# gersteinlab/REPIC-copy

Hardware: AMD Instinct MI355X
Metric: micrographs/sec (get_cliques, whole node) at 1/2/4/8 MI355X; % HBM roofline (higher is better)
Workload: dtype f64; 1 GPU; C2: {'k': 3, 'n_true': 300, 'box': 180, 'width': 4096, 'height': 4096, 'keep': 0.9, 'jit': 0.08, 'fp': 0.1}; micrographs_per_gpu=10000, scaling=weak, k=3, box_size=180, boxes_per_gpu=9030947, edges_per_gpu=11401310, cliques_per_gpu=5244495, parallelism=dp1 (micrograph shards), io=HBM-resident, steps_in_flight=3, streams=3

## Files before the change

repic-copy_amd/csrc/rgc_abi.cpp:

```cpp
#include <hip/hip_runtime_api.h>

#include <algorithm>
#include <climits>
#include <cstdio>
#include <cstdlib>
#include <cstring>
#include <string>
#include <map>
#include <mutex>
#include <thread>
#include <tuple>
#include <vector>

#include "../../include/repic_gc.h"
#include "pyset.h"
#include "rgc_kernels.h"

using namespace rgc;

static thread_local std::string g_err;

static int fail(const std::string& msg) {
  g_err = msg;
  return -1;
// ... 1 lines not shown
#define HIPCHK(expr)                                                                   \
  do {                                                                                 \
    hipError_t e_ = (expr);                                                            \
    if (e_ != hipSuccess)                                                              \
      return fail(std::string(#expr) + ": " + hipGetErrorString(e_));                   \
  } while (0)
#define TRY(expr)           \
  do {                      \
    int r_ = (expr);        \
    if (r_ != 0) return r_; \
  } while (0)

namespace {

enum DevBufId {
  D_FBOXOFF, D_FIDBASE, D_MGLIST, D_MGOUT, D_CURSOR, D_X, D_Y, D_S,
  D_ROWS, D_W, D_CONF, D_CONS, D_MEMBERS, D_ORDER,
  D_SUBMG, D_SUBX, D_SUBY, D_SUBS, D_ORIG, D_STAMPS,
  D_BOXOFF, D_CELLOFF, D_P0OFF, D_IDBASE, D_GRID, D_CELLSTART, D_SX, D_SY, D_SBOX, D_SPICK, D_SMG, D_BMG,
  D_BPICK, D_FWDCNT, D_FWDOFF, D_TILES, D_TOTAL, D_EDST, D_EJI, D_PARENT, D_HASEDGE, D_CSIZE,
  D_STAT, D_INSKEY, D_COMPMIN, D_CCOUNT, D_COFF, D_INCL, D_VLIST, D_VSORT, D_VROW, D_BOFF, D_RLO, D_ADJG, D_RBOUND, D_RFLAG, D_DFSMG, D_ROOTBOX, D_EXLIST,
  D_LCNT, D_LOFF, D_LROOT0, D_LROOT1, D_LM0, D_LM1, D_LP0, D_LP1, D_PK,
  D_QG, D_QGSLOT,
  D_TIES,
  D_EU, D_EV, D_EJIOUT,
  D_SC_BOX, D_SC_GOFF, D_SC_POFF, D_SC_TP, D_SC_TR, D_SC_TW, D_SC_CNT,
  D_IL_CPTR, D_IL_ROW, D_IL_W, D_IL_REP, D_IL_PAR, D_IL_ROOT, D_IL_CSIZE, D_IL_RCNT, D_IL_RCUR,
  D_IL_RPTR, D_IL_RCOLS, D_IL_CID, D_IL_CN, D_IL_COFF, D_IL_CCUR, D_IL_MEM, D_IL_LOC, D_IL_SCR,
  D_IL_BIG, D_IL_NBIG, D_IL_WSCR, D_IL_X, D_IL_EX, D_IL_RLOC, D_IL_CERT, D_IL_KEY, D_IL_ST,
  D_IL_RMAX, D_IL_OWN, D_IL_LAM, D_IL_GRAD, D_IL_CS, D_IL_CNT, D_IL_GAP, D_IL_STSAVE,
  D_IL_FS, D_IL_FSCNT, D_IL_FSKEEP, D_LBUCKET, D_WIDELIST,
  D_PK_META, D_PK_COLMG, D_PK_SEL, D_PK_SELCNT, D_PK_PRIMAL, D_PK_OFF, D_PK_X, D_PK_PX, D_PK_PY,
  D_PK_PCONF, D_PK_PCOL, D_PK_CONF, D_PK_CX, D_PK_CY,
  D_COUNT
};
enum HostBufId {
  H_FSTAGE, H_STAGE, H_TOTAL, H_MGOUT, H_STAT, H_MGOFF, H_ROWS, H_W, H_CONF, H_CONS, H_MEMBERS,
  H_ORDER, H_EU, H_EV, H_EJIOUT,
  H_PK_META, H_PK_MG, H_PK_PX, H_PK_PY, H_PK_PCONF, H_PK_PCOL, H_COUNT
};

struct Buf {
  void* p = nullptr;
  size_t cap = 0;
};

constexpr int LDS_BLOCK = 1280;
// ... 123 lines not shown
  std::string pend_err;
  int64_t fix_fetch_bytes = 0;
};

static int ensure_dev(rgc_ctx* c, int id, size_t bytes, size_t keep = 0) {
  Buf& b = c->d[id];
  if (bytes == 0) bytes = 16;
  if (b.cap >= bytes) return 0;
  size_t cap = std::max(bytes, b.cap + b.cap / 2);
  cap = (cap + 255) & ~(size_t)255;
  void* p = nullptr;
  HIPCHK(hipMalloc(&p, cap));
  if (b.p && keep) {
    HIPCHK(hipMemcpyAsync(p, b.p, std::min(keep, b.cap), hipMemcpyDeviceToDevice, c->stream));
    HIPCHK(hipStreamSynchronize(c->stream));
  }
  if (b.p) HIPCHK(hipFree(b.p));
  b.p = p;
  b.cap = cap;
  if (id == D_TILES) {
    HIPCHK(hipMemsetAsync(p, 0, cap, c->stream));
    c->tiles_epoch = scan_epoch_count();
  }
  return 0;
}

static int tiles_refresh(rgc_ctx* c) {
  Buf& b = c->d[D_TILES];
  if (!b.p || scan_epoch_count() - c->tiles_epoch < SCAN_EPOCH_REFRESH) return 0;
  HIPCHK(hipMemsetAsync(b.p, 0, b.cap, c->stream));
  c->tiles_epoch = scan_epoch_count();
  return 0;
}

constexpr int QG_BYTES = 1 << 20;
static int ensure_qg(rgc_ctx* c, FusedArgs& A, int k, int nt) {
  A.qg_base = nullptr;
  A.qg_slots = nullptr;
  A.qg_nslots = 0;
  A.qg_bytes = 0;
  if (nt != 1024 || k != 4) return 0;
  if (!c->qg_nslots) {
    int ncu = 0;
    HIPCHK(hipDeviceGetAttribute(&ncu, hipDeviceAttributeMultiprocessorCount, c->device));
    const int ns = (2 * std::max(ncu, 1) + 31) / 32 * 32;
    TRY(ensure_dev(c, D_QG, (size_t)ns * QG_BYTES));
// ... 44 lines not shown
                          bool multi) {
  TRY(ensure_dev(c, D_ROWS, need * k * 4, keep * k * 4));
  TRY(ensure_dev(c, D_W, need * 4, keep * 4));
  TRY(ensure_dev(c, D_CONF, need * 4, keep * 4));
  TRY(ensure_dev(c, D_CONS, need * 4, keep * 4));
  TRY(ensure_dev(c, D_TIES, need * (4 + k) * 4));
  if (members) TRY(ensure_dev(c, D_MEMBERS, need * k * 4, keep * k * 4));
  if (multi) TRY(ensure_dev(c, D_ORDER, need * k, keep * k));
  return 0;
}

static int ensure_edges(rgc_ctx* c, int64_t need, int64_t keep) {
  TRY(ensure_dev(c, D_EU, need * 4, keep * 4));
  TRY(ensure_dev(c, D_EV, need * 4, keep * 4));
  TRY(ensure_dev(c, D_EJIOUT, need * 8, keep * 8));
  return 0;
}

struct FusedIo {
  unsigned long long *cur, *clear;
  const unsigned long long* h_cur;
  int slot;
  MgOut o;
};
static int fused_io(rgc_ctx* c, int n_mg, size_t cur_off, FusedIo* io) {
  TRY(ensure_host(c, H_MGOUT, cur_off + 2 * CUR_BYTES));
  TRY(ensure_dev(c, D_MGOUT, cur_off + 2 * CUR_BYTES));
  char* d = D<char>(c, D_MGOUT);
  if (c->slots_at != d || c->slots_off != cur_off) {
    HIPCHK(hipMemsetAsync(d + cur_off, 0, 2 * CUR_BYTES, c->stream));
    c->slots_at = d;
    c->slots_off = cur_off;
    c->cur_slot = 0;
  }
  const int sl = c->cur_slot;
  io->slot = sl;
  io->cur = reinterpret_cast<unsigned long long*>(d + cur_off + sl * CUR_BYTES);
  io->clear = reinterpret_cast<unsigned long long*>(d + cur_off + (1 - sl) * CUR_BYTES);
  io->h_cur = reinterpret_cast<const unsigned long long*>(H<char>(c, H_MGOUT) + cur_off +
                                                           sl * CUR_BYTES);
  io->o = mgout_bind(d, n_mg);
  return 0;
}

static int run_multi(rgc_ctx* c, int n_mg, int k, double B, double two_b2, int get_cc, int multi,
                     bool want_members, bool want_ji, const int64_t* box_off, const int64_t* id_base, const double* x,
                     const double* y, const double* sc, int64_t out_base,
                     std::vector<MgStat>& st_out, int64_t* C_out, int64_t* E_out) {
  const int64_t N = box_off[(int64_t)n_mg * k];
  const size_t nbo = (size_t)n_mg * k + 1;
  std::vector<int32_t> cell_off(n_mg + 1);
  int64_t cells = 0;
  bool bin_wide = false;
  int max_n = 0;
  for (int m = 0; m < n_mg; ++m) {
    const int64_t nm = box_off[(int64_t)(m + 1) * k] - box_off[(int64_t)m * k];
    bin_wide |= nm > 65535;
    max_n = std::max<int>(max_n, (int)std::min<int64_t>(nm, INT32_MAX));
  }
  for (int m = 0; m < n_mg; ++m) {
    cell_off[m] = (int32_t)cells;
    const int64_t nm = box_off[(int64_t)(m + 1) * k] - box_off[(int64_t)m * k];
    cells += bin_budget(nm, bin_wide) + 2;
  }
// ... 391 lines not shown
      if (want_edges) TRY(ensure_edges(c, c->cap_edges, 0));
      FusedIo io;
      TRY(fused_io(c, n_mg, cur_off, &io));
      if (attempt > 0) HIPCHK(hipMemsetAsync(io.cur, 0, CUR_BYTES, s));
      h_cur = io.h_cur;
      FusedArgs A{};
      A.k = k; A.flags = get_cc | (multi << 1) | (want_members ? 32 : 0);
      A.B = B; A.two_b2 = two_b2;
      A.box_off = d_bo; A.id_base = d_id;
      A.x = x; A.y = y; A.score = sc; A.o = io.o;
      A.cursor = io.cur; A.cap = c->cap_cliques;
      A.cursor_clear = io.clear;
      A.rows = D<int32_t>(c, D_ROWS); A.w = D<float>(c, D_W); A.conf = D<float>(c, D_CONF);
      A.consensus = D<int32_t>(c, D_CONS);
      A.members = want_members ? D<int32_t>(c, D_MEMBERS) : nullptr;
      A.order = multi ? D<uint8_t>(c, D_ORDER) : nullptr;
      A.stamps = nullptr;
      A.eu = want_edges ? D<int32_t>(c, D_EU) : nullptr;
      A.ev = want_edges ? D<int32_t>(c, D_EV) : nullptr;
      A.eji = want_edges ? D<double>(c, D_EJIOUT) : nullptr;
      A.ecap_out = c->cap_edges;
      A.tie_list = D<int32_t>(c, D_TIES);
      A.tie_cap = c->cap_cliques;
      A.esum_n = 0;
      A.wide_list = nullptr;
      A.mg_count = nullptr;
      int64_t ties_done = 0;
#ifdef RGC_STAMPS
      TRY(ensure_dev(c, D_STAMPS, 3 * (size_t)n_mg * rgc::STAMP_SLOTS * 8));
      HIPCHK(hipMemsetAsync(D<void>(c, D_STAMPS), 0, 3 * (size_t)n_mg * rgc::STAMP_SLOTS * 8, s));
#endif
      std::vector<int32_t> todo = todo0, left;
      int ml_off = 0;
      bool overflow = false;
      for (int pass = 0; pass < 3 && (!todo.empty() || (pass == 0 && all0)); ++pass) {
        const bool wide = pass > 0;
        const bool single = pass == 0 && all0;
        std::vector<int> keys;
        std::vector<std::vector<int32_t>> lists;
        left.clear();
        if (single) {
          keys.assign(1, fused_class(nmaxb));
          lists.assign(1, std::vector<int32_t>());
        }
        int last = -1;
        for (int32_t m : todo) {
          const int cl = mg_class(m);
          if (!cl || !plan_of(pass, cl).nmax) { left.push_back(m); continue; }
          if (last < 0 || keys[last] != cl) {
            last = -1;
// ... 17 lines not shown
            HIPCHK(hipMemcpyAsync(D<int32_t>(c, D_MGLIST) + ml_off, f_ml + ml_off, by.size() * 4,
                                  hipMemcpyHostToDevice, s));
        }
        for (size_t q = 0; q < keys.size(); ++q) {
          const FusedPlan& pl = plan_of(pass, keys[q]);
          A.nmax = pl.nmax;
          A.ecap = pl.ecap;
          A.mg_list = single ? nullptr : D<int32_t>(c, D_MGLIST) + ml_off + starts[q];
#ifdef RGC_STAMPS
          A.stamps = D<unsigned long long>(c, D_STAMPS) + (size_t)(ml_off + starts[q]) * rgc::STAMP_SLOTS;
#endif
          TRY(ensure_qg(c, A, k, pl.nt));
          TRY(mark(c, "k_fused"));
          const int le = launch_fused(s, single ? n_mg : (int)lists[q].size(), pl.lds, A, wide,
                                      pl.nt);
          if (le != 0)
            return fail(std::string("fused kernel launch failed (k=") + std::to_string(k) +
                        (wide ? ", f64" : ", f32") + " layout, nmax " + std::to_string(pl.nmax) +
                        ", lds " + std::to_string(pl.lds) + ", " +
                        std::to_string(pl.nt) + " threads): " +
                        (le > 0 ? hipGetErrorString((hipError_t)le) : "unsupported k"));
        }
        TRY(mark(c, "k_fused_ties"));
        if (launch_fused_ties(s, A, ties_done) != 0) return fail("tie kernel launch failed");
        TRY(mark(c, "d2h_stats"));
        HIPCHK(hipMemcpyAsync(H<void>(c, H_MGOUT), D<void>(c, D_MGOUT), cur_off + 2 * CUR_BYTES,
                              hipMemcpyDeviceToHost, s));
        if (c->timing) {
          if (!c->ev_tail) HIPCHK(hipEventCreate(&c->ev_tail));
          HIPCHK(hipEventRecord(c->ev_tail, s));
        }
        HIPCHK(hipGetLastError());
        HIPCHK(hipStreamSynchronize(s));
        const int32_t* fst = ho.status;
        ties_done = std::min<int64_t>((int64_t)h_cur[rgc::CUR_TIES], A.tie_cap);
        ml_off += (int)by.size();
        todo.clear();
        auto check = [&](int32_t m) {
          const int stt = fst[m];
          if (stt == RGC_ST_OVERFLOW) overflow = true;
          else if (stt == RGC_ST_DEFER_WIDE || stt == RGC_ST_DEFER) todo.push_back(m);
        };
        if (single) {
          for (int32_t m = 0; m < n_mg; ++m)
            if (fst[m] >= RGC_ST_DEFER) check(m);
        } else {
          for (const int32_t m : by) check(m);
        }
        for (int32_t m : left) todo.push_back(m);
      }
      fused_total = (int64_t)h_cur[0];
      c->cur_slot = 1 - c->cur_slot;
#ifdef RGC_STAMPS
      const size_t n0w = all0 ? (size_t)n_mg : todo0.size();
      c->stamps.resize(n0w * rgc::STAMP_SLOTS);
      HIPCHK(hipMemcpy(c->stamps.data(), D<void>(c, D_STAMPS), n0w * rgc::STAMP_SLOTS * 8,
                       hipMemcpyDeviceToHost));
#endif
// ... 229 lines not shown
  if (c->cap_cliques < 4096) c->cap_cliques = std::max<int64_t>(4096, N);
  TRY(ensure_outputs(c, c->cap_cliques, 0, k, want_members, multi));
  FusedIo io;
  TRY(fused_io(c, n_mg, cur_off, &io));
  FusedArgs A{};
  A.k = k;
  A.flags = ((flags & RGC_F_GET_CC) ? 1 : 0) | (multi ? 2 : 0) | (want_members ? 32 : 0);
  A.B = (double)in->box_size;
  A.two_b2 = (double)(2 * in->box_size * in->box_size);
  A.box_off = in->dev_box_off; A.id_base = in->dev_id_base;
  A.x = in->x; A.y = in->y; A.score = in->score;
  A.o = io.o;
  A.cursor = io.cur; A.cap = c->cap_cliques;
  A.cursor_clear = io.clear;
  A.rows = D<int32_t>(c, D_ROWS); A.w = D<float>(c, D_W); A.conf = D<float>(c, D_CONF);
  A.consensus = D<int32_t>(c, D_CONS);
  A.members = want_members ? D<int32_t>(c, D_MEMBERS) : nullptr;
  A.order = multi ? D<uint8_t>(c, D_ORDER) : nullptr;
  A.stamps = nullptr;
  A.eu = nullptr; A.ev = nullptr; A.eji = nullptr; A.ecap_out = 0;
  A.mg_list = nullptr;
  A.tie_list = D<int32_t>(c, D_TIES);
  A.tie_cap = c->cap_cliques;
  A.esum_n = n_mg;
  A.mg_count = nullptr;
  const FusedPlan* pw = c->wide_hint ? &cached_plan(k, 1, fused_class(nmaxb)) : nullptr;
  if (pw && !pw->nmax) pw = nullptr;
  A.wide_list = nullptr;
  if (pw) {
    TRY(ensure_dev(c, D_WIDELIST, (size_t)n_mg * 4));
    A.wide_list = D<int32_t>(c, D_WIDELIST);
  }
#ifdef RGC_STAMPS
  return 0;
#endif
  int32_t* d_ml = nullptr;
  if (grp.size() > 1) {
    TRY(ensure_host(c, H_FSTAGE, (size_t)n_mg * 4));
    TRY(ensure_dev(c, D_MGLIST, (size_t)n_mg * 4));
    int32_t* h_ml = H<int32_t>(c, H_FSTAGE);
    size_t o = 0;
    for (const auto& g : grp) {
      std::memcpy(h_ml + o, g.mg.data(), g.mg.size() * 4);
      o += g.mg.size();
    }
    d_ml = D<int32_t>(c, D_MGLIST);
// ... 13 lines not shown
    if (le != 0) return fail("fused kernel launch failed (submit): " +
                             std::string(le > 0 ? hipGetErrorString((hipError_t)le) : "unsupported k"));
  }
  if (pw) {
    FusedArgs Aw = A;
    Aw.mg_list = A.wide_list;
    Aw.mg_count = io.cur + 5;
    Aw.wide_list = nullptr;
    Aw.nmax = pw->nmax;
    Aw.ecap = pw->ecap;
    TRY(ensure_qg(c, Aw, k, pw->nt));
    TRY(mark(c, "k_fused"));
    const int le = launch_fused(s, n_mg, pw->lds, Aw, true, pw->nt);
    if (le != 0) return fail("fused f64 kernel launch failed (submit): " +
                             std::string(le > 0 ? hipGetErrorString((hipError_t)le) : "unsupported k"));
  }
  const bool stats_in_ties = !(flags & RGC_F_LAZY_STATS) && A.tie_list && A.tie_cap > 0;
  if (stats_in_ties) {
    A.stats_dev = D<char>(c, D_MGOUT);
    A.host_stats = H<char>(c, H_MGOUT);
    A.stats_bytes = (int64_t)cur_off;
  }
  TRY(mark(c, "k_fused_ties"));
  if (launch_fused_ties(s, A, 0) != 0) return fail("tie kernel launch failed (submit)");
  c->pend_slot = io.slot;
  c->cur_slot = 1 - c->cur_slot;
  if (c->timing) {
    if (!c->ev_tail) HIPCHK(hipEventCreate(&c->ev_tail));
    HIPCHK(hipEventRecord(c->ev_tail, s));
  }
  if (!c->ev_sub) HIPCHK(hipEventCreateWithFlags(&c->ev_sub, hipEventDisableTiming));
  if (stats_in_ties || (flags & RGC_F_LAZY_STATS)) {
    const size_t so = cur_off + (size_t)io.slot * CUR_BYTES;
    HIPCHK(hipMemcpyAsync(H<char>(c, H_MGOUT) + so, D<char>(c, D_MGOUT) + so, CUR_BYTES,
                          hipMemcpyDeviceToHost, s));
    HIPCHK(hipEventRecord(c->ev_sub, s));
  } else {
    if (!c->copy_set) {
      TRY(shared_copy_stream(c->device, &c->copy_stream));
      c->copy_set = true;
    }
    if (!c->ev_k) HIPCHK(hipEventCreateWithFlags(&c->ev_k, hipEventDisableTiming));
    HIPCHK(hipEventRecord(c->ev_k, s));
    HIPCHK(hipStreamWaitEvent(c->copy_stream, c->ev_k, 0));
    HIPCHK(hipMemcpyAsync(H<void>(c, H_MGOUT), D<void>(c, D_MGOUT), cur_off + 2 * CUR_BYTES,
                          hipMemcpyDeviceToHost, c->copy_stream));
    HIPCHK(hipEventRecord(c->ev_sub, c->copy_stream));
// ... 973 lines not shown
```

repic-copy_amd/csrc/rgc_fused.hip:

```cpp
#pragma clang fp contract(off)

#include <type_traits>

#ifdef RGC_STAMPS
#include <hip/hip_runtime.h>
namespace rgc {
__shared__ unsigned long long g_bwait[16];
__device__ __forceinline__ void raw_barrier() {
  __builtin_amdgcn_fence(__ATOMIC_RELEASE, "workgroup");
  __builtin_amdgcn_s_barrier();
  __builtin_amdgcn_fence(__ATOMIC_ACQUIRE, "workgroup");
}
__device__ __forceinline__ void timed_barrier() {
  const unsigned long long t0 = __builtin_amdgcn_s_memtime();
  raw_barrier();
  if ((threadIdx.x & 63) == 0) g_bwait[threadIdx.x >> 6] += __builtin_amdgcn_s_memtime() - t0;
}
}
#define __syncthreads() ::rgc::timed_barrier()
#endif

#include "rgc_device.h"
#include "rgc_kernels.h"

// ... 1 lines not shown

constexpr int MAXW = 16;
constexpr int fused_rb(int nt) { return nt <= 256 ? 4 : nt >= 1024 ? 5 : 2; }
constexpr int fused_rq(int nt) { return nt >= 1024 ? 0 : fused_rb(nt); }
constexpr int fused_rv(int nt) { return nt >= 1024 ? 0 : fused_rb(nt); }

struct FusedHdr {
  union {
    struct {
      double redd[MAXW];
      int64_t red64[MAXW];
      uint64_t redu[MAXW];
      int redi[MAXW];
    };
    double red4[4][MAXW];
  };
  double minx, miny, cell, inv_cell, inv_celly;
  double xbs;
  float inv_gy;
  int gx, gy, ncell, nkey;
  int E, nodes, cc_cnt, cc_max, target, V, status;
  uint32_t ccur;
  int tief[2];
  int qslot;
  int64_t C, base;
};

__host__ __device__ inline int fused_cells(int nmax) { return nmax <= 2048 ? 4 * nmax : 2 * nmax; }

__host__ __device__ inline int fwd_blocks(int nmax) { return (nmax + 63) / 64; }

__host__ __device__ inline FusedLayout fused_layout(int nmax, int ecap, bool wide) {
  FusedLayout L;
  auto al = [](int v) { return (v + 15) & ~15; };
  int o = al((int)sizeof(FusedHdr));
  L.off_sxy = o; o += al((wide ? 16 : 8) * nmax);
  L.off_cnt = o; o += al(4 * (nmax + 4));
  L.off_fwd = o; o += al(2 * (fwd_blocks(nmax) * 65 + 4));
  L.off_pos = o; o += al(2 * nmax);
  L.off_vrank = o; o += al(2 * nmax);
  L.off_dst = o; o += al(2 * ecap);
  L.off_union = o;
  L.off_cstart = o; o += al(2 * (fused_cells(nmax) + 8));
  L.off_parent = o; o += al(2 * (nmax + 8));
  L.off_scell = o; o += al(2 * nmax);
  L.off_citems = o; o += al(2 * nmax);
// ... 49 lines not shown
  double B, two_b2;
  float Bf, two_b2f;
  int flags;
  gptr<const double> score;
  gptr<int32_t> rows;
  gptr<float> w;
  gptr<float> conf;
  gptr<int32_t> consensus;
  gptr<int32_t> members;
  gptr<uint8_t> order;
  FShared S;
  int pb[K + 1];
  int pp[K + 1];
  int m, b0, n;
  int64_t idb;
  bool set_order;
  int64_t out;
  int64_t c0, c1;
  int64_t count;
  uint16_t* cq_ord;
  uint32_t* ccur;
  int cq_cap;
  gptr<int32_t> tie_list;
  gptr<unsigned long long> tie_count;
  int64_t tie_cap;
};

__device__ __forceinline__ uint32_t lds_ld(uint32_t* p) {
  return __hip_atomic_load(p, __ATOMIC_RELAXED, __HIP_MEMORY_SCOPE_WORKGROUP);
}
__device__ __forceinline__ void lds_st(uint32_t* p, uint32_t v) {
  __hip_atomic_store(p, v, __ATOMIC_RELAXED, __HIP_MEMORY_SCOPE_WORKGROUP);
}
__device__ __forceinline__ uint32_t p16_ld(uint16_t* p) {
  return __hip_atomic_load(p, __ATOMIC_RELAXED, __HIP_MEMORY_SCOPE_WORKGROUP);
}
__device__ __forceinline__ void p16_st(uint16_t* p, uint32_t v) {
  __hip_atomic_store(p, (uint16_t)v, __ATOMIC_RELAXED, __HIP_MEMORY_SCOPE_WORKGROUP);
}
__device__ __forceinline__ uint32_t uf_find_lds(uint16_t* parent, uint32_t x) {
  for (;;) {
    const uint32_t p = p16_ld(parent + x);
    if (p == x) return x;
    const uint32_t gp = p16_ld(parent + p);
    if (gp != p) p16_st(parent + x, gp);
    x = gp;
  }
}
// ... 228 lines not shown
      } else {
        const double a = (double)Is[NE / 2 - 1], b = (double)Is[NE / 2];
        med = ((a / (c.two_b2 - a)) + (b / (c.two_b2 - b))) / 2.0;
      }
    } else if (NE & 1) {
      med = median_n<NE>(Is);
      med = med / (c.two_b2 - med);
    } else {
      bool nan = false;
#pragma unroll
      for (int t = 0; t < NE; ++t) nan |= isnan(Is[t]);
      mid_n<NE>(Is);
      const double a = Is[NE / 2 - 1], b = Is[NE / 2];
      med = nan ? NAN : ((a / (c.two_b2 - a)) + (b / (c.two_b2 - b))) / 2.0;
    }
    const float conf32 = (float)cf;
    c.w[j] = (float)((double)conf32 * med);
    c.conf[j] = conf32;
  }
  if (c.flags & (2 | 32)) {
#pragma unroll
    for (int i = 0; i < K; ++i) c.members[j * K + i] = c.b0 + li[i];
  }
  if (c.flags & 2) return true;
  float deg[K];
#pragma unroll
  for (int i = 0; i < K; ++i) deg[i] = 0.0f;
  {
    int t = 0;
#pragma unroll
    for (int a = 0; a < K; ++a)
#pragma unroll
      for (int b = a + 1; b < K; ++b) {
        float jf;
        if constexpr (INTP) jf = I[t] * __builtin_amdgcn_rcpf(c.two_b2f - I[t]);
        else jf = (float)I[t] * __builtin_amdgcn_rcpf((float)(c.two_b2 - I[t]));
        deg[a] += jf;
        deg[b] += jf;
        ++t;
      }
  }
  float d1 = deg[0], d2 = -INFINITY;
  int arg = 0;
#pragma unroll
  for (int i = 1; i < K; ++i) {
    const float d = deg[i];
    d2 = d > d1 ? d1 : fmaxf(d2, d);
    arg = d > d1 ? i : arg;
    d1 = fmaxf(d1, d);
  }
  if (!(d1 - d2 > 3e-5f)) return true;
  int cons = li[0];
#pragma unroll
  for (int i = 1; i < K; ++i) cons = (arg == i) ? li[i] : cons;
  c.consensus[j] = c.b0 + cons;
  return false;
}

template <int K, bool W>
__device__ __forceinline__ void fused_epilogue_order(const FCtx<K>& c, int64_t j,
                                                     const int (&mem)[K]) {
  double ji[K][K], xs[K], ys[K];
  int li[K];
  uint64_t ins[K] = {};
#pragma unroll
  for (int i = 0; i < K; ++i) {
    const double2 xy = ld_xy<W>(c.S, mem[i]);
    xs[i] = xy.x;
    ys[i] = xy.y;
    li[i] = c.S.citems[mem[i]];
  }
#pragma unroll
  for (int a = 0; a < K; ++a)
#pragma unroll
    for (int b = a + 1; b < K; ++b) ji[a][b] = jaccard(xs[a], ys[a], xs[b], ys[b], c.B, c.two_b2);
  if (!c.set_order) {
    for (int i = 0; i < K; ++i) ins[i] = ins_key<K>(c, mem[i]);
  }
  uint32_t top;
  int arg = epi_degree_max<K>(ji, &top);
  const bool tie = (top & (top - 1)) != 0;
  const bool multi = (c.flags & 2) != 0;
  if (tie || multi) {
    if (c.set_order) {
      const unsigned long long t = atomicAdd((unsigned long long*)c.tie_count, 1ull);
      if ((int64_t)t < c.tie_cap) {
        gptr<int32_t> e = c.tie_list + (int64_t)t * (4 + K);
        e[0] = (int32_t)(uint32_t)(uint64_t)j;
        e[1] = (int32_t)(uint32_t)((uint64_t)j >> 32);
        e[2] = c.m;
        e[3] = (int32_t)(top | (tie ? 0x10000u : 0u) | (multi ? 0x20000u : 0u));
#pragma unroll
        for (int i = 0; i < K; ++i) e[4 + i] = c.b0 + li[i];
      }
      if (tie) return;
    } else {
      const uint32_t ord = node_order_ins<K>(ins);
      if (tie) arg = epi_tie_arg<K>(top, ord);
      if (multi) {
#pragma unroll
        for (int i = 0; i < K; ++i) c.order[j * K + i] = (uint8_t)((ord >> (4 * i)) & 15);
      }
    }
  }
  int cons = li[0];
#pragma unroll
  for (int i = 1; i < K; ++i) cons = (arg == i) ? li[i] : cons;
  c.consensus[j] = c.b0 + cons;
}

template <int K, int D, bool FILL>
struct FLevel {
  __device__ __forceinline__ static void run(FCtx<K>& c, int (&mem)[K]) {
    const int prev = mem[D - 1];
    const int lo = c.S.eb(prev);
    int hi;
    if (FILL) hi = lb16(c.S.dst, lo, c.S.ee(prev), c.pp[D + 1]);
    else hi = c.S.split[prev];
    for (int e = lo; e < hi; ++e) {
      const int h = c.S.dst[e];
      bool ok = true;
#pragma unroll
      for (int q = 0; q < D - 1; ++q) {
        if (!contains16(c.S.dst, c.S.eb(mem[q]), c.S.ee(mem[q]), h)) { ok = false; break; }
      }
// ... 630 lines not shown
  do {                                            \
    if ((ph) == RGC_STOP_AFTER) {                 \
      if (tid == 0) put_stats(A, m, 0, 0, 0, 0, 0, 0, 0, 0); \
      return;                                     \
    }                                             \
  } while (0)
#else
#define STOP_AFTER(ph) \
  do {                 \
  } while (0)
#endif
  STAMP(0);
#ifdef RGC_STAMPS
  const uint32_t rt0 = (uint32_t)__builtin_amdgcn_s_memrealtime();
#endif
  FCtx<K> c;
  c.B = sdetach(A.B); c.two_b2 = sdetach(A.two_b2); c.flags = sdetach(A.flags);
  c.score = gdetach(A.score);
  c.Bf = uff((float)A.B);
  c.two_b2f = uff((float)A.two_b2);
  c.rows = gdetach(A.rows); c.w = gdetach(A.w); c.conf = gdetach(A.conf);
  c.consensus = gdetach(A.consensus);
  c.members = gdetach(A.members); c.order = gdetach(A.order);
  c.tie_list = gdetach(A.tie_list); c.tie_count = gdetach(A.cursor) + CUR_TIES;
  c.tie_cap = sdetach(A.tie_cap);
  const gptr<const double> ax = gdetach(A.x);
  const gptr<const double> ay = gdetach(A.y);
  c.S = S;
  c.m = m;
  c.b0 = A.box_off[m * K];
  c.n = A.box_off[m * K + K] - c.b0;
#pragma unroll
  for (int i = 0; i <= K; ++i) c.pb[i] = A.box_off[m * K + i] - c.b0;
  c.idb = A.id_base[m];
  const int n = c.n, b0 = c.b0;

  constexpr int RB = fused_rb(NT);
  constexpr int RQ = fused_rq(NT), RV = fused_rv(NT);
  double rx[RB], ry[RB];
#pragma unroll
  for (int j = 0; j < RB; ++j) {
    const int i = tid + j * FWG;
    rx[j] = i < n ? ax[b0 + i] : 0.0;
    ry[j] = i < n ? ay[b0 + i] : 0.0;
  }
  auto each_box = [&](auto&& fn) {
#pragma unroll
    for (int j = 0; j < RB; ++j) {
// ... 67 lines not shown
            gx = fx; gy = fy;
            break;
          }
          fch *= 1.0625f;
        }
        cl = (double)fch;
        icly = (double)__builtin_amdgcn_rcpf(fch);
        icl = 0.5 * icly;
        if (icl * (1.08 * A.B) > 1.0) icl = 1.0 / (1.08 * A.B);
        if (icly * (0.54 * A.B) > 1.0) icly = 1.0 / (0.54 * A.B);
      }
    }
    if (tid == 0) {
      const double ex = mxx - mnx;
      H.minx = mnx; H.miny = mny; H.cell = cl; H.inv_cell = icl; H.inv_celly = icly;
      H.gx = gx; H.gy = gy;
      H.ncell = gx * gy; H.nkey = K * gx * gy;
      H.inv_gy = gy > 0 ? __builtin_amdgcn_rcpf((float)gy) : 0.0f;
      H.xbs = (mnx < mxx && ex < 0x1p60) ? (double)((float)n * __builtin_amdgcn_rcpf((float)ex))
                                         : 0.0;
      H.status = (!W && mnx == -INFINITY) ? RGC_ST_DEFER_WIDE : 0;
      H.C = 0; H.base = 0; H.V = 0; H.target = -1; H.ccur = 0; H.E = 0;
      H.tief[0] = H.tief[1] = 0;
      H.qslot = 0;
    }
  }
  __syncthreads();
  if (!W && H.status == RGC_ST_DEFER_WIDE) {
    if (tid == 0) put_stats(A, m, RGC_ST_DEFER_WIDE, 0, 0, 0, 0, 0, 0, 0);
    return;
  }
  const GridU G = grid_u(H);
  const int nk = G.nkey;
  uint32_t* cw = reinterpret_cast<uint32_t*>(S.cstart);
  auto count_box = [&](int i, double xv, double yv) {
    const int q = box_key<W>(G, picker_of<K>(c.pb, i), xv, yv);
    const uint32_t t = atomicAdd(&cw[q >> 1], 1u << (16 * (q & 1)));
    return (uint32_t)q | (((t >> (16 * (q & 1))) & 0xFFFFu) << 16);
  };
  auto park = [&](int i, uint32_t v) {
    S.pos[i] = (uint16_t)(v & 0xFFFFu);
    S.citems[i] = (uint16_t)(v >> 16);
  };
  uint32_t rq[RQ > 0 ? RQ : 1];
#pragma unroll
  for (int j = 0; j < RB; ++j) {
// ... 446 lines not shown
    __syncthreads();
    const bool overflow = H.base + H.C > A.cap;
    if (overflow && tid == 0) H.status = RGC_ST_OVERFLOW;

    STOP_AFTER(5);
    STAMP(10);
    if (!overflow) {
    c.S.vstaged = 8 * H.V <= L.off_citems - L.off_parent;
    if (c.S.vstaged) {
      for (int t = tid; t < n; t += FWG) {
        const int f = S.flags[t], vr = S.vrank[t], li = S.citems[t];
        if (f != 3) continue;
        c.S.vscore[vr] = c.score[b0 + li];
      }
      __syncthreads();
    }

    STAMP(11);
    const int Cm = ufl((int)H.C);
    const int cap = ufl(c.cq_cap);
    const int64_t obase = (int64_t)(((uint64_t)(uint32_t)ufl((int)(H.base >> 32)) << 32) |
                                    (uint32_t)ufl((int)H.base));
    const int nit = bfs_ok ? nch : (Cm + cap - 1) / cap;
    BfsOut<K> cur = bo;
    for (int ci = 0; ci < nit; ++ci) {
      int c0, c1;
      if (tid == 0) H.tief[(ci + 1) & 1] = 0;
      if (bfs_ok) {
        const int ch = ci == 0 ? nch - 1 : ci - 1;
        c0 = ufl((int)chtab[2 * ch + 1]);
        c1 = ufl((int)chtab[2 * ch + 3]);
        if constexpr (K >= 4) {
          if (ci > 0)
            cur = we ? bfs_cliques<K, true, NT, QG && K <= 4>(S, H, q, qbytes, ufl((int)chtab[2 * ch]),
                                       ufl((int)chtab[2 * ch + 2]), get_cc, (uint32_t)target,
                                       tid, c.pp, ep)
                     : bfs_cliques<K, true, NT>(S, H, q, qbytes, ufl((int)chtab[2 * ch]),
                                       ufl((int)chtab[2 * ch + 2]), get_cc, (uint32_t)target,
                                       tid, c.pp, ep);
        }
        c.cq_ord = reinterpret_cast<uint16_t*>(q + cur.lvl[K] + (we ? 8 : 4) * (c1 - c0));
      } else {
        c0 = ci * cap;
        c1 = min(Cm, c0 + cap);
        c.c0 = c0;
        c.c1 = c1;
// ... 44 lines not shown
            const uint2 v = nx;
            if (sl + FWG < cnt) nx = ent[sl + FWG];
            const int t[4] = {(int)(v.x & 0xFFFF), (int)(v.x >> 16), (int)(v.y & 0xFFFF),
                              (int)(v.y >> 16)};
            int mem[K];
#pragma unroll
            for (int i = 0; i < K; ++i) mem[i] = t[i];
            epi(sl, mem);
          }
        } else {
          for (int sl = tid; sl < c1 - c0; sl += FWG) {
            int mem[K];
            clique_members(sl, mem);
            epi(sl, mem);
          }
        }
      } else {
        for (int sl = tid; sl < c1 - c0; sl += FWG) {
          int mem[K];
          clique_members(sl, mem);
          epi(sl, mem);
        }
      }
      if (any) H.tief[ci & 1] = 1;
      __syncthreads();
      if (H.tief[ci & 1]) {
        for (int sl = tid; sl < c1 - c0; sl += FWG) {
          if (!order_flag(sl)) continue;
          int mem[K];
          const int64_t jo = clique_members(sl, mem);
          fused_epilogue_order<K, W>(c, jo, mem);
        }
      }
      __syncthreads();
    }
    }
  }
  STAMP(12);
#ifdef RGC_STAMPS
  if (tid == 0)
    A.stamps[(int64_t)blockIdx.x * STAMP_SLOTS + 13] =
        ((unsigned long long)(uint32_t)__builtin_amdgcn_s_memrealtime() << 32) | rt0;
#endif
  if constexpr (QG) {
    if (qslot >= 0) {
      __syncthreads();
      if (tid == 0) {
        __threadfence();
        atomicAnd(A.qg_slots + (qslot >> 5), ~(1u << (qslot & 31)));
      }
    }
  }
  if (tid == 0)
    put_stats(A, m, H.status, H.E, H.nodes, H.cc_cnt, H.cc_max, H.V, H.base, H.C);
}

template <int K>
__global__ __launch_bounds__(256) void k_fused_ties(FusedArgs A, int64_t from) {
  if (A.esum_n > 0 && blockIdx.x < 16) {
    __shared__ int64_t red[4];
    int64_t e = 0;
    for (int m = blockIdx.x * 256 + threadIdx.x; m < A.esum_n; m += 16 * 256) {
      const int st = A.o.status[m];
      if (st == 0 || st == RGC_ST_NO_CLIQUES || st == RGC_ST_NO_EDGES) e += A.o.n_edges[m];
    }
    e = block_sum64<256>(e, red);
    if (threadIdx.x == 0 && e) atomicAdd(A.cursor + 1, (unsigned long long)e);
  }
  const int64_t n = min((int64_t)__hip_atomic_load(A.cursor + CUR_TIES, __ATOMIC_RELAXED,
                                                    __HIP_MEMORY_SCOPE_AGENT), A.tie_cap);
  for (int64_t t = from + (int64_t)blockIdx.x * 256 + threadIdx.x; t < n;
       t += (int64_t)gridDim.x * 256) {
    const int32_t* e = A.tie_list + t * (4 + K);
    const int64_t j = (int64_t)(((uint64_t)(uint32_t)e[1] << 32) | (uint32_t)e[0]);
    const int m = e[2];
    const uint32_t fl = (uint32_t)e[3];
    const int64_t idb = A.id_base[m] - (int64_t)A.box_off[m * K];
    int mem[K];
    double xs[K], ys[K];
    int64_t ids[K];
    const uint64_t ins[K] = {};
#pragma unroll
    for (int i = 0; i < K; ++i) {
      mem[i] = e[4 + i];
      xs[i] = A.x[mem[i]];
      ys[i] = A.y[mem[i]];
      ids[i] = idb + mem[i];
    }
    const uint32_t ord = node_order<K>(mem, xs, ys, ids, true, ins);
    if (fl & 0x10000u) A.consensus[j] = mem[epi_tie_arg<K>(fl & 0xFFFFu, ord)];
    if (fl & 0x20000u) {
#pragma unroll
      for (int i = 0; i < K; ++i) A.order[j * K + i] = (uint8_t)((ord >> (4 * i)) & 15);
    }
  }
  if (A.host_stats) {
    const int64_t n16 = A.stats_bytes / 16;
    const uint4* src = reinterpret_cast<const uint4*>(A.stats_dev);
    uint4* dst = reinterpret_cast<uint4*>(A.host_stats);
    for (int64_t i = (int64_t)blockIdx.x * 256 + threadIdx.x; i < n16; i += (int64_t)gridDim.x * 256)
      dst[i] = src[i];
  }
}

int launch_fused_ties(hipStream_t stream, const FusedArgs& A, int64_t from) {
  if (!A.tie_list || A.tie_cap <= from) return 0;
  const dim3 g(256), b(256);
  switch (A.k) {
#define RGC_TIES_CASE(KK) \
  case KK: hipLaunchKernelGGL((k_fused_ties<KK>), g, b, 0, stream, A, from); break;
    RGC_TIES_CASE(2) RGC_TIES_CASE(3) RGC_TIES_CASE(4) RGC_TIES_CASE(5) RGC_TIES_CASE(6)
    RGC_TIES_CASE(7) RGC_TIES_CASE(8)
#undef RGC_TIES_CASE
    default:
      return -1;
  }
  return (int)hipGetLastError();
}

template <int K, bool W, int NT, bool QG = false>
static int launch_fused_t(hipStream_t stream, int n_blocks, int lds_bytes, const FusedArgs& A) {
  static std::atomic<uint64_t> attr_set{0};
#ifdef RGC_STAMPS
  constexpr int kStaticLds = 256;
#else
  constexpr int kStaticLds = 0;
#endif
  const hipError_t e = set_dyn_lds_once(attr_set, reinterpret_cast<const void*>(&k_fused<K, W, NT, QG>),
                                        160 * 1024 - kStaticLds);
  if (e != hipSuccess) return (int)e;
  hipLaunchKernelGGL((k_fused<K, W, NT, QG>), dim3(n_blocks), dim3(NT), lds_bytes, stream, A);
  return (int)hipGetLastError();
}
// ... 80 lines not shown
```

repic-copy_amd/csrc/rgc_kernels.h:

```cpp
#pragma once
#include <hip/hip_runtime.h>
#include <stdint.h>

#include <atomic>

namespace rgc {

inline hipError_t set_dyn_lds_once(std::atomic<uint64_t>& done, const void* fn, int bytes) {
  int dev = 0;
  hipError_t e = hipGetDevice(&dev);
  if (e != hipSuccess) return e;
  const uint64_t bit = dev < 64 ? (1ULL << dev) : 0;
  if (bit && (done.load(std::memory_order_acquire) & bit)) return hipSuccess;
  e = hipFuncSetAttribute(fn, hipFuncAttributeMaxDynamicSharedMemorySize, bytes);
  if (e == hipSuccess && bit) done.fetch_or(bit, std::memory_order_acq_rel);
  return e;
}

constexpr int MAX_K = 8;
constexpr int SCAN_TILE = 2048;

struct MgGrid {
  double minx, miny, cell, inv_cell, inv_celly;
  int gx, gy, ncell, nkey, flags, pad;
};
__host__ __device__ inline int bin_budget(int64_t n, bool wide) {
  const int64_t cap = wide ? 32760 : 65528;
  return (int)(2 * n + 64 < cap ? 2 * n + 64 : cap);
}

struct MgStat {
  int64_t n_edges;
  int64_t clique_base, clique_cnt;
  int n_nodes, cc_cnt, cc_max, status, target, n_vert;
};

constexpr int CUR_TIES = 8;

constexpr int RGC_ST_NO_EDGES = 1;
constexpr int RGC_ST_NO_CLIQUES = 2;
constexpr int RGC_ST_DEFER = 3;
constexpr int RGC_ST_OVERFLOW = 4;
constexpr int RGC_ST_DEFER_WIDE = 5;

struct FusedLayout {
  int off_sxy, off_cnt, off_fwd, off_pos, off_vrank, off_dst, off_union, off_cstart, off_parent,
      off_citems, off_scell, off_flags, off_smark, off_cbuf, total;
};

struct MgOut {
  int32_t* status;
  int32_t* cc_max;
  int32_t* cc_cnt;
  int32_t* n_nodes;
  int32_t* n_vert;
  int64_t* n_edges;
  int64_t* clique_base;
  int64_t* clique_cnt;
};
inline size_t mgout_bytes(int n_mg) { return (size_t)n_mg * 20 + 8 + (size_t)n_mg * 24; }
// ... 23 lines not shown
  const double* x;
  const double* y;
  const double* score;
  MgOut o;
  unsigned long long* cursor;
  unsigned long long* cursor_clear;
  int64_t cap;
  int32_t* rows;
  float* w;
  float* conf;
  int32_t* consensus;
  int32_t* members;
  uint8_t* order;
  unsigned long long* stamps;
  int32_t* eu;
  int32_t* ev;
  double* eji;
  int64_t ecap_out;
  char* qg_base;
  uint32_t* qg_slots;
  int qg_nslots, qg_bytes;
  int32_t* tie_list;
  int64_t tie_cap;
  int esum_n;
  int32_t* wide_list;
  const unsigned long long* mg_count;
  const char* stats_dev;
  char* host_stats;
  int64_t stats_bytes;
};

int fused_lds_bytes(int nmax, int ecap, bool wide);
int fused_vgprs(int k, bool wide, int nt);
bool fused_nt_ok(int k, int nt);
int launch_fused(hipStream_t stream, int n_blocks, int lds_bytes, const FusedArgs& A, bool wide,
                 int nt);
int launch_fused_ties(hipStream_t stream, const FusedArgs& A, int64_t from);
void launch_gather(hipStream_t stream, int n_sub, int k, const int32_t* sub_mg,
                   const int32_t* box_off, const int32_t* sub_box_off, const double* x,
                   const double* y, const double* s, double* ox, double* oy, double* os,
                   int32_t* orig);
void launch_remap(hipStream_t stream, int64_t C, int k, const int32_t* orig, int32_t* consensus,
                  int32_t* members);
void launch_dump_edges(hipStream_t stream, int N, const int64_t* fwd_off, const int32_t* e_dst,
                       const double* e_ji, const int32_t* orig, int32_t* eu, int32_t* ev,
                       double* eji);

constexpr int RB_W = 64;

struct CliqueArgs {
  int k;
  int flags;
  int n_mg, n_roots;
  int64_t C;
  double B, two_b2;
  const int32_t* box_off;
  const int32_t* p0off;
  const int64_t* id_base;
  const double* x;
  const double* y;
// ... 191 lines not shown
```

Measured before the change: 30.56 million micrographs/s.

## Replace global tie queue with per-micrograph LDS tie counters and segmented resolve

Switches tie and multi-order deferral from a single global 64-bit atomic queue to a per-block LDS counter, writing compact entries into the clique's own output range. The per-micrograph count is stored in a device array, and the tie kernel resolves entries with a wave-level prefix scan and binary search over micrographs. The deferred path now recomputes the Jaccard degree and consensus for every handed-off clique. The goal is to remove global atomic contention and the host-side ties_done bookkeeping, at the cost of more work in the tie kernel and an extra per-micrograph counter buffer that the kernel clears after reading.

```diff
diff --git a/repic-copy_amd/csrc/rgc_abi.cpp b/repic-copy_amd/csrc/rgc_abi.cpp
--- a/repic-copy_amd/csrc/rgc_abi.cpp
+++ b/repic-copy_amd/csrc/rgc_abi.cpp
@@ -47,7 +47,7 @@
   D_STAT, D_INSKEY, D_COMPMIN, D_CCOUNT, D_COFF, D_INCL, D_VLIST, D_VSORT, D_VROW, D_BOFF, D_RLO, D_ADJG, D_RBOUND, D_RFLAG, D_DFSMG, D_ROOTBOX, D_EXLIST,
   D_LCNT, D_LOFF, D_LROOT0, D_LROOT1, D_LM0, D_LM1, D_LP0, D_LP1, D_PK,
   D_QG, D_QGSLOT,
-  D_TIES,
+  D_TIES, D_TIECNT,
   D_EU, D_EV, D_EJIOUT,
   D_SC_BOX, D_SC_GOFF, D_SC_POFF, D_SC_TP, D_SC_TR, D_SC_TW, D_SC_CNT,
   D_IL_CPTR, D_IL_ROW, D_IL_W, D_IL_REP, D_IL_PAR, D_IL_ROOT, D_IL_CSIZE, D_IL_RCNT, D_IL_RCUR,
@@ -217,6 +217,7 @@
     HIPCHK(hipMemsetAsync(p, 0, cap, c->stream));
     c->tiles_epoch = scan_epoch_count();
   }
+  if (id == D_TIECNT) HIPCHK(hipMemsetAsync(p, 0, cap, c->stream));
   return 0;
 }
 
@@ -307,6 +308,7 @@
   const unsigned long long* h_cur;
   int slot;
   MgOut o;
+  int32_t* tie_cnt;
 };
 static int fused_io(rgc_ctx* c, int n_mg, size_t cur_off, FusedIo* io) {
   TRY(ensure_host(c, H_MGOUT, cur_off + 2 * CUR_BYTES));
@@ -325,6 +327,8 @@
   io->h_cur = reinterpret_cast<const unsigned long long*>(H<char>(c, H_MGOUT) + cur_off +
                                                            sl * CUR_BYTES);
   io->o = mgout_bind(d, n_mg);
+  TRY(ensure_dev(c, D_TIECNT, (size_t)n_mg * 4));
+  io->tie_cnt = D<int32_t>(c, D_TIECNT);
   return 0;
 }
 
@@ -762,10 +766,11 @@
       A.ecap_out = c->cap_edges;
       A.tie_list = D<int32_t>(c, D_TIES);
       A.tie_cap = c->cap_cliques;
+      A.tie_cnt = io.tie_cnt;
+      A.tie_n = n_mg;
       A.esum_n = 0;
       A.wide_list = nullptr;
       A.mg_count = nullptr;
-      int64_t ties_done = 0;
 #ifdef RGC_STAMPS
       TRY(ensure_dev(c, D_STAMPS, 3 * (size_t)n_mg * rgc::STAMP_SLOTS * 8));
       HIPCHK(hipMemsetAsync(D<void>(c, D_STAMPS), 0, 3 * (size_t)n_mg * rgc::STAMP_SLOTS * 8, s));
@@ -829,7 +834,7 @@
                         (le > 0 ? hipGetErrorString((hipError_t)le) : "unsupported k"));
         }
         TRY(mark(c, "k_fused_ties"));
-        if (launch_fused_ties(s, A, ties_done) != 0) return fail("tie kernel launch failed");
+        if (launch_fused_ties(s, A) != 0) return fail("tie kernel launch failed");
         TRY(mark(c, "d2h_stats"));
         HIPCHK(hipMemcpyAsync(H<void>(c, H_MGOUT), D<void>(c, D_MGOUT), cur_off + 2 * CUR_BYTES,
                               hipMemcpyDeviceToHost, s));
@@ -840,7 +845,6 @@
         HIPCHK(hipGetLastError());
         HIPCHK(hipStreamSynchronize(s));
         const int32_t* fst = ho.status;
-        ties_done = std::min<int64_t>((int64_t)h_cur[rgc::CUR_TIES], A.tie_cap);
         ml_off += (int)by.size();
         todo.clear();
         auto check = [&](int32_t m) {
@@ -1116,6 +1120,8 @@
   A.mg_list = nullptr;
   A.tie_list = D<int32_t>(c, D_TIES);
   A.tie_cap = c->cap_cliques;
+  A.tie_cnt = io.tie_cnt;
+  A.tie_n = n_mg;
   A.esum_n = n_mg;
   A.mg_count = nullptr;
   const FusedPlan* pw = c->wide_hint ? &cached_plan(k, 1, fused_class(nmaxb)) : nullptr;
@@ -1175,7 +1181,7 @@
     A.stats_bytes = (int64_t)cur_off;
   }
   TRY(mark(c, "k_fused_ties"));
-  if (launch_fused_ties(s, A, 0) != 0) return fail("tie kernel launch failed (submit)");
+  if (launch_fused_ties(s, A) != 0) return fail("tie kernel launch failed (submit)");
   c->pend_slot = io.slot;
   c->cur_slot = 1 - c->cur_slot;
   if (c->timing) {
diff --git a/repic-copy_amd/csrc/rgc_fused.hip b/repic-copy_amd/csrc/rgc_fused.hip
--- a/repic-copy_amd/csrc/rgc_fused.hip
+++ b/repic-copy_amd/csrc/rgc_fused.hip
@@ -47,6 +47,7 @@
   int E, nodes, cc_cnt, cc_max, target, V, status;
   uint32_t ccur;
   int tief[2];
+  uint32_t tiec;
   int qslot;
   int64_t C, base;
 };
@@ -142,8 +143,8 @@
   uint32_t* ccur;
   int cq_cap;
   gptr<int32_t> tie_list;
-  gptr<unsigned long long> tie_count;
-  int64_t tie_cap;
+  int64_t tie_base;
+  uint32_t* tiec;
 };
 
 __device__ __forceinline__ uint32_t lds_ld(uint32_t* p) {
@@ -418,7 +419,16 @@
 #pragma unroll
     for (int i = 0; i < K; ++i) c.members[j * K + i] = c.b0 + li[i];
   }
-  if (c.flags & 2) return true;
+  auto hand_off = [&]() -> bool {
+    if (!c.set_order) return true;
+    const uint32_t t = atomicAdd(c.tiec, 1u);
+    gptr<int32_t> e = c.tie_list + (c.tie_base + t) * (1 + K);
+    e[0] = (int32_t)(j - c.tie_base);
+#pragma unroll
+    for (int i = 0; i < K; ++i) e[1 + i] = c.b0 + li[i];
+    return false;
+  };
+  if (c.flags & 2) return hand_off();
   float deg[K];
 #pragma unroll
   for (int i = 0; i < K; ++i) deg[i] = 0.0f;
@@ -445,7 +455,7 @@
     arg = d > d1 ? i : arg;
     d1 = fmaxf(d1, d);
   }
-  if (!(d1 - d2 > 3e-5f)) return true;
+  if (!(d1 - d2 > 3e-5f)) return hand_off();
   int cons = li[0];
 #pragma unroll
   for (int i = 1; i < K; ++i) cons = (arg == i) ? li[i] : cons;
@@ -458,7 +468,7 @@
                                                      const int (&mem)[K]) {
   double ji[K][K], xs[K], ys[K];
   int li[K];
-  uint64_t ins[K] = {};
+  uint64_t ins[K];
 #pragma unroll
   for (int i = 0; i < K; ++i) {
     const double2 xy = ld_xy<W>(c.S, mem[i]);
@@ -470,33 +480,17 @@
   for (int a = 0; a < K; ++a)
 #pragma unroll
     for (int b = a + 1; b < K; ++b) ji[a][b] = jaccard(xs[a], ys[a], xs[b], ys[b], c.B, c.two_b2);
-  if (!c.set_order) {
-    for (int i = 0; i < K; ++i) ins[i] = ins_key<K>(c, mem[i]);
-  }
+  for (int i = 0; i < K; ++i) ins[i] = ins_key<K>(c, mem[i]);
   uint32_t top;
   int arg = epi_degree_max<K>(ji, &top);
   const bool tie = (top & (top - 1)) != 0;
   const bool multi = (c.flags & 2) != 0;
   if (tie || multi) {
-    if (c.set_order) {
-      const unsigned long long t = atomicAdd((unsigned long long*)c.tie_count, 1ull);
-      if ((int64_t)t < c.tie_cap) {
-        gptr<int32_t> e = c.tie_list + (int64_t)t * (4 + K);
-        e[0] = (int32_t)(uint32_t)(uint64_t)j;
-        e[1] = (int32_t)(uint32_t)((uint64_t)j >> 32);
-        e[2] = c.m;
-        e[3] = (int32_t)(top | (tie ? 0x10000u : 0u) | (multi ? 0x20000u : 0u));
-#pragma unroll
-        for (int i = 0; i < K; ++i) e[4 + i] = c.b0 + li[i];
-      }
-      if (tie) return;
-    } else {
-      const uint32_t ord = node_order_ins<K>(ins);
-      if (tie) arg = epi_tie_arg<K>(top, ord);
-      if (multi) {
-#pragma unroll
-        for (int i = 0; i < K; ++i) c.order[j * K + i] = (uint8_t)((ord >> (4 * i)) & 15);
-      }
+    const uint32_t ord = node_order_ins<K>(ins);
+    if (tie) arg = epi_tie_arg<K>(top, ord);
+    if (multi) {
+#pragma unroll
+      for (int i = 0; i < K; ++i) c.order[j * K + i] = (uint8_t)((ord >> (4 * i)) & 15);
     }
   }
   int cons = li[0];
@@ -1173,8 +1167,9 @@
   c.rows = gdetach(A.rows); c.w = gdetach(A.w); c.conf = gdetach(A.conf);
   c.consensus = gdetach(A.consensus);
   c.members = gdetach(A.members); c.order = gdetach(A.order);
-  c.tie_list = gdetach(A.tie_list); c.tie_count = gdetach(A.cursor) + CUR_TIES;
-  c.tie_cap = sdetach(A.tie_cap);
+  c.tie_list = gdetach(A.tie_list);
+  c.tie_base = 0;
+  c.tiec = &H.tiec;
   const gptr<const double> ax = gdetach(A.x);
   const gptr<const double> ay = gdetach(A.y);
   c.S = S;
@@ -1288,6 +1283,7 @@
       H.status = (!W && mnx == -INFINITY) ? RGC_ST_DEFER_WIDE : 0;
       H.C = 0; H.base = 0; H.V = 0; H.target = -1; H.ccur = 0; H.E = 0;
       H.tief[0] = H.tief[1] = 0;
+      H.tiec = 0;
       H.qslot = 0;
     }
   }
@@ -1780,6 +1776,7 @@
     const int64_t obase = (int64_t)(((uint64_t)(uint32_t)ufl((int)(H.base >> 32)) << 32) |
                                     (uint32_t)ufl((int)H.base));
     const int nit = bfs_ok ? nch : (Cm + cap - 1) / cap;
+    c.tie_base = obase;
     BfsOut<K> cur = bo;
     for (int ci = 0; ci < nit; ++ci) {
       int c0, c1;
@@ -1870,6 +1867,10 @@
           epi(sl, mem);
         }
       }
+      if (c.set_order) {
+        __syncthreads();
+        continue;
+      }
       if (any) H.tief[ci & 1] = 1;
       __syncthreads();
       if (H.tief[ci & 1]) {
@@ -1882,6 +1883,7 @@
       }
       __syncthreads();
     }
+    if (tid == 0 && H.tiec) A.tie_cnt[m] = (int32_t)H.tiec;
     }
   }
   STAMP(12);
@@ -1904,7 +1906,7 @@
 }
 
 template <int K>
-__global__ __launch_bounds__(256) void k_fused_ties(FusedArgs A, int64_t from) {
+__global__ __launch_bounds__(256) void k_fused_ties(FusedArgs A) {
   if (A.esum_n > 0 && blockIdx.x < 16) {
     __shared__ int64_t red[4];
     int64_t e = 0;
@@ -1915,31 +1917,78 @@
     e = block_sum64<256>(e, red);
     if (threadIdx.x == 0 && e) atomicAdd(A.cursor + 1, (unsigned long long)e);
   }
-  const int64_t n = min((int64_t)__hip_atomic_load(A.cursor + CUR_TIES, __ATOMIC_RELAXED,
-                                                    __HIP_MEMORY_SCOPE_AGENT), A.tie_cap);
-  for (int64_t t = from + (int64_t)blockIdx.x * 256 + threadIdx.x; t < n;
-       t += (int64_t)gridDim.x * 256) {
-    const int32_t* e = A.tie_list + t * (4 + K);
-    const int64_t j = (int64_t)(((uint64_t)(uint32_t)e[1] << 32) | (uint32_t)e[0]);
-    const int m = e[2];
-    const uint32_t fl = (uint32_t)e[3];
-    const int64_t idb = A.id_base[m] - (int64_t)A.box_off[m * K];
-    int mem[K];
-    double xs[K], ys[K];
-    int64_t ids[K];
-    const uint64_t ins[K] = {};
-#pragma unroll
-    for (int i = 0; i < K; ++i) {
-      mem[i] = e[4 + i];
-      xs[i] = A.x[mem[i]];
-      ys[i] = A.y[mem[i]];
-      ids[i] = idb + mem[i];
-    }
-    const uint32_t ord = node_order<K>(mem, xs, ys, ids, true, ins);
-    if (fl & 0x10000u) A.consensus[j] = mem[epi_tie_arg<K>(fl & 0xFFFFu, ord)];
-    if (fl & 0x20000u) {
-#pragma unroll
-      for (int i = 0; i < K; ++i) A.order[j * K + i] = (uint8_t)((ord >> (4 * i)) & 15);
+  const int lane = threadIdx.x & 63;
+  const int nw = (int)gridDim.x * 4, wv = (int)blockIdx.x * 4 + ((int)threadIdx.x >> 6);
+  const int n_mg = A.tie_n;
+  const int G = min(64, max(1, (n_mg + nw - 1) / nw));
+  const bool multi = (A.flags & 2) != 0;
+  for (int64_t g0 = (int64_t)wv * G; g0 < n_mg; g0 += (int64_t)nw * G) {
+    const int ml = (int)g0 + lane;
+    int cnt = 0, blo = 0, bhi = 0;
+    if (lane < G && ml < n_mg) {
+      const int64_t base = A.o.clique_base[ml];
+      cnt = A.tie_cnt[ml];
+      blo = (int)(uint32_t)(uint64_t)base;
+      bhi = (int)(uint32_t)((uint64_t)base >> 32);
+      if (cnt) A.tie_cnt[ml] = 0;
+    }
+    int inc = cnt;
+#pragma unroll
+    for (int d = 1; d < 64; d <<= 1) {
+      const int v = __shfl_up(inc, d, 64);
+      if (lane >= d) inc += v;
+    }
+    const int T = __shfl(inc, 63, 64);
+    for (int e0 = 0; e0 < T; e0 += 64) {
+      const bool act = e0 + lane < T;
+      const int en = min(e0 + lane, T - 1);
+      int lo = 0, hi = 63;
+#pragma unroll
+      for (int st = 0; st < 6; ++st) {
+        const int mid = (lo + hi) >> 1;
+        const bool up = __shfl(inc, mid, 64) > en;
+        hi = up ? mid : hi;
+        lo = up ? lo : mid + 1;
+      }
+      const int t = en - (__shfl(inc, lo, 64) - __shfl(cnt, lo, 64));
+      const int64_t base = (int64_t)(((uint64_t)(uint32_t)__shfl(bhi, lo, 64) << 32) |
+                                     (uint32_t)__shfl(blo, lo, 64));
+      if (!act) continue;
+      const int m = (int)g0 + lo;
+      const int32_t* e = A.tie_list + (base + t) * (1 + K);
+      const int64_t j = base + e[0];
+      const int64_t idb = A.id_base[m] - (int64_t)A.box_off[m * K];
+      int mem[K];
+      double xs[K], ys[K], ji[K][K];
+      int64_t ids[K];
+      const uint64_t ins[K] = {};
+#pragma unroll
+      for (int i = 0; i < K; ++i) {
+        mem[i] = e[1 + i];
+        xs[i] = A.x[mem[i]];
+        ys[i] = A.y[mem[i]];
+        ids[i] = idb + mem[i];
+      }
+#pragma unroll
+      for (int a = 0; a < K; ++a)
+#pragma unroll
+        for (int b = a + 1; b < K; ++b)
+          ji[a][b] = jaccard(xs[a], ys[a], xs[b], ys[b], A.B, A.two_b2);
+      uint32_t top;
+      int arg = epi_degree_max<K>(ji, &top);
+      const bool tie = (top & (top - 1)) != 0;
+      if (tie || multi) {
+        const uint32_t ord = node_order<K>(mem, xs, ys, ids, true, ins);
+        if (tie) arg = epi_tie_arg<K>(top, ord);
+        if (multi) {
+#pragma unroll
+          for (int i = 0; i < K; ++i) A.order[j * K + i] = (uint8_t)((ord >> (4 * i)) & 15);
+        }
+      }
+      int cons = mem[0];
+#pragma unroll
+      for (int i = 1; i < K; ++i) cons = (arg == i) ? mem[i] : cons;
+      A.consensus[j] = cons;
     }
   }
   if (A.host_stats) {
@@ -1951,12 +2000,12 @@
   }
 }
 
-int launch_fused_ties(hipStream_t stream, const FusedArgs& A, int64_t from) {
-  if (!A.tie_list || A.tie_cap <= from) return 0;
-  const dim3 g(256), b(256);
+int launch_fused_ties(hipStream_t stream, const FusedArgs& A) {
+  if (!A.tie_list || !A.tie_cnt || A.tie_cap <= 0) return 0;
+  const dim3 g((unsigned)std::min(1024, std::max(256, (A.tie_n + 3) / 4))), b(256);
   switch (A.k) {
 #define RGC_TIES_CASE(KK) \
-  case KK: hipLaunchKernelGGL((k_fused_ties<KK>), g, b, 0, stream, A, from); break;
+  case KK: hipLaunchKernelGGL((k_fused_ties<KK>), g, b, 0, stream, A); break;
     RGC_TIES_CASE(2) RGC_TIES_CASE(3) RGC_TIES_CASE(4) RGC_TIES_CASE(5) RGC_TIES_CASE(6)
     RGC_TIES_CASE(7) RGC_TIES_CASE(8)
 #undef RGC_TIES_CASE
diff --git a/repic-copy_amd/csrc/rgc_kernels.h b/repic-copy_amd/csrc/rgc_kernels.h
--- a/repic-copy_amd/csrc/rgc_kernels.h
+++ b/repic-copy_amd/csrc/rgc_kernels.h
@@ -34,8 +34,6 @@
   int64_t clique_base, clique_cnt;
   int n_nodes, cc_cnt, cc_max, status, target, n_vert;
 };
-
-constexpr int CUR_TIES = 8;
 
 constexpr int RGC_ST_NO_EDGES = 1;
 constexpr int RGC_ST_NO_CLIQUES = 2;
@@ -105,6 +103,8 @@
   int qg_nslots, qg_bytes;
   int32_t* tie_list;
   int64_t tie_cap;
+  int32_t* tie_cnt;
+  int tie_n;
   int esum_n;
   int32_t* wide_list;
   const unsigned long long* mg_count;
@@ -118,7 +118,7 @@
 bool fused_nt_ok(int k, int nt);
 int launch_fused(hipStream_t stream, int n_blocks, int lds_bytes, const FusedArgs& A, bool wide,
                  int nt);
-int launch_fused_ties(hipStream_t stream, const FusedArgs& A, int64_t from);
+int launch_fused_ties(hipStream_t stream, const FusedArgs& A);
 void launch_gather(hipStream_t stream, int n_sub, int k, const int32_t* sub_mg,
                    const int32_t* box_off, const int32_t* sub_box_off, const double* x,
                    const double* y, const double* s, double* ox, double* oy, double* os,
```

After: 30.46 million micrographs/s. Within noise of the previous version (-0.3%).
